# marcottelab/FluorosequencingImageAnalysis

Hardware: AMD Instinct MI355X
Metric: psf_lm_fits_per_sec (higher is better)
Workload: dtype f64

## Files before the change

fluorosequencingimageanalysis_amd/csrc/fsq_fit_rounds.hip:

```cpp
#include <algorithm>
#include <atomic>
#include <cstdlib>

#include <mutex>
#include <new>
#include <type_traits>
#include <vector>

#include "fsq_common.h"
#include "fsq_lm_quad.h"
#include "fsq_evalguard.h"
#include "fsq_kb_tilemap.h"

namespace {

#define WAVE_SYNC() do { __builtin_amdgcn_fence(__ATOMIC_RELEASE, "wavefront"); __builtin_amdgcn_wave_barrier(); \
                         __builtin_amdgcn_fence(__ATOMIC_ACQUIRE, "wavefront"); } while (0)

#ifdef FSQ_DEBUG_HZ
__device__ unsigned long long g_hz[32];
#endif
#ifdef FSQ_PHASE_PROFILE
__device__ unsigned long long g_rphase[32];
#define RPH_DECL unsigned long long rph_t0 = clock64(), rph_acc[16] = {0,0,0,0,0,0,0,0,0,0,0,0,0,0,0,0};
#define RPH_MARK(k) { unsigned long long t_ = clock64(); rph_acc[k] += t_ - rph_t0; rph_t0 = t_; }
#define RPH_FLUSH(off) if (threadIdx.x == 0 && (blockIdx.x & 63) == 0) { for (int k_ = 0; k_ < 16; k_++) atomicAdd(&g_rphase[(off) + k_], rph_acc[k_]); }
#else
#define RPH_DECL
#define RPH_MARK(k)
#define RPH_FLUSH(off)
#endif

enum { CNT_LINE = 32, CNT_A = 0, CNT_B0 = CNT_LINE, CNT_C1 = CNT_B0 + KB_C1 * CNT_LINE, CNT_C3 = CNT_B0 + KB_C3 * CNT_LINE,
       CNT_KINDS = 1 + KB_LISTS, CNT_SET = 8 * CNT_LINE };
__host__ __device__ inline int cnt_of_list(int list) { return CNT_B0 + list * CNT_LINE; }
enum { Q_EPS = Q_WA3 };
enum { A_IDX = 0, A_X = 1, A_DIAG = 8, A_LLIM1 = 15, A_FNORM = 16, A_PAR = 17, A_DELTA = 18, A_XNORM = 19, A_ITER = 20,
       A_HDR = 21 , A_E = 21 , A_LEN = 46,
       B_GNORM = 21, B_IPVT = 22, B_QTF = 23, B_SDIAG = 30, B_R = 37, B_LEN = 65,
       C_PARL = 65, C_PARU = 66, C_FP = 67, C_LMIT = 68, C_LEN = 69 };

struct FitOut {
    double x[FSQ_NP];
    int status, niter, nfev, pad;
};
struct FitStat {
    double vmax, vmean;
};

struct Ctx {
    uint16_t* roi;
    int pix32;
    FitOut* out;
    FitStat* stat;
    long long cap;
    long long pool;
    int* err;
    int* slow_total;
    int* done;
    int tshift;
    int wave_prio;
    int force_redo;
    int force_slow_mod;
};

enum { G_KINIT_POS = 1, G_KINIT_SLOT = 2, G_KA_B = 3, G_KA_OVERLAP = 5, G_KA_SLOW = 6, G_KB_C1 = 7, G_KB_C3 = 8, G_KB_A = 9,
       G_KB_B = 10 };
FSQ_DEV long long fsq_guard(const Ctx& c, long long v, long long limit, int code)
{
    if ((unsigned long long)v < (unsigned long long)limit) return v;
    atomicMax(c.err, code);
    return 0;
}

FSQ_DEV int wave_reserve(int* counter, bool want)
{
    const unsigned long long m = __ballot(want);
    if (m == 0) return 0;
    const int lane = threadIdx.x & 63;
    const int leader = __ffsll((long long)m) - 1;
    int base = 0;
    if (lane == leader) base = atomicAdd(counter, __popcll(m));
    base = __shfl(base, leader);
    return base + __popcll(m & ((1ull << lane) - 1ull));
}

FSQ_DEV int wave_reserve4(int* counters, bool want, int list, int* other)
{
    const int lane = threadIdx.x & 63;
    unsigned long long m[4];
#pragma unroll
    for (int l = 0; l < 4; l++) m[l] = __ballot(want && list == l);
    const unsigned long long mine = list == 0 ? m[0] : list == 1 ? m[1] : list == 2 ? m[2] : m[3];
    const unsigned long long pair = list == 0 ? m[1] : list == 1 ? m[0] : list == 2 ? m[3] : m[2];
    const int leader = want ? __ffsll((long long)mine) - 1 : lane;
    int base = 0;
    if (want && lane == leader) base = atomicAdd(counters + list * CNT_LINE, __popcll(mine));
    const int pair_base = __shfl(base, pair ? __ffsll((long long)pair) - 1 : lane);
    base = __shfl(base, leader);
    *other = pair ? pair_base + __popcll(pair) : 0;
    return want ? base + __popcll(mine & ((1ull << lane) - 1ull)) : 0;
}

FSQ_DEV long long wave_reserve_checked(const Ctx& c, int* counter, bool want, long long limit, int code)
{
    const int at = wave_reserve(counter, want);
    return want ? fsq_guard(c, at, limit, code) : 0;
}

struct BatchArgs {
    const uint16_t* src; const int32_t* cand; int H, W; long long n; int from_image;
    int pix_fmt;
    long long base;
    int ticket;
    int no_queue;
};

FSQ_DEV void wave_mark_done(int* done, bool term, int ticket)
{
    unsigned long long m = __ballot(term);
    const int lane = threadIdx.x & 63;
    while (m) {
        const int leader = __ffsll((long long)m) - 1;
        const int t = __shfl(ticket, leader);
        const unsigned long long mm = __ballot(term && ticket == t);
        if (lane == leader) atomicAdd(done + t, __popcll(mm));
        m &= ~mm;
    }
}

#ifndef FSQ_NT
#define FSQ_NT 0
#endif
typedef unsigned fsq_u4v __attribute__((ext_vector_type(4)));
FSQ_DEV double nt_ld(const double* p) { return FSQ_NT ? __builtin_nontemporal_load(p) : *p; }
FSQ_DEV void nt_st(double* p, double v) { if (FSQ_NT) __builtin_nontemporal_store(v, p); else *p = v; }
FSQ_DEV uint4 nt_ld4(const void* p)
{
    const fsq_u4v v = FSQ_NT ? __builtin_nontemporal_load((const fsq_u4v*)p) : *(const fsq_u4v*)p;
    return make_uint4(v.x, v.y, v.z, v.w);
}
FSQ_DEV void nt_st4(void* p, uint4 w)
{
    fsq_u4v v; v.x = w.x; v.y = w.y; v.z = w.z; v.w = w.w;
    if (FSQ_NT) __builtin_nontemporal_store(v, (fsq_u4v*)p); else *(fsq_u4v*)p = v;
}
struct NtRef {
    double* p;
    FSQ_DEV operator double() const { return nt_ld(p); }
    FSQ_DEV void operator=(double v) const { nt_st(p, v); }
};
struct NtQ {
    double* p;
    FSQ_DEV NtRef operator[](long long i) const { return NtRef{p + i}; }
};
FSQ_DEV NtQ ntq(const double* p) { return NtQ{const_cast<double*>(p)}; }

FSQ_DEV int tag_slot(const Ctx& c, int tag) { return (int)((unsigned)tag & ((1u << c.tshift) - 1u)); }
FSQ_DEV int tag_ticket(const Ctx& c, int tag) { return (int)((unsigned)tag >> c.tshift); }

FSQ_DEV int rpk(int i, int k) { return i * 7 - (i * (i - 1)) / 2 + (k - i); }
FSQ_DEV double pack2(int a, int b) { return __longlong_as_double(((long long)(unsigned)a) | ((long long)b << 32)); }
FSQ_DEV void unpack2(double v, int* a, int* b) { long long u = __double_as_longlong(v); *a = (int)(unsigned)(u & 0xffffffffll); *b = (int)(u >> 32); }

FSQ_DEV void roi_pixels(const BatchArgs& c, long long idx, double* d)
{
    if (c.from_image) {
        const int f = c.cand[3 * idx], h = c.cand[3 * idx + 1], w = c.cand[3 * idx + 2];
        const size_t base = ((size_t)f * c.H + (h - 2)) * c.W + (w - 2);
#pragma unroll
        for (int a = 0; a < 5; a++)
#pragma unroll
            for (int b = 0; b < 5; b++) d[a * 5 + b] = (double)fsq_pixel(c.src, base + (size_t)a * c.W + b, c.pix_fmt);
    } else {
#pragma unroll
        for (int k = 0; k < FSQ_NPIX; k++) d[k] = (double)c.src[idx * FSQ_NPIX + k];
    }
}

FSQ_DEV void roi_compact(const Ctx& c, long long idx, double* d)
{
    if (c.pix32) {
        const uint32_t* s32 = (const uint32_t*)c.roi + (size_t)idx * 32;
#pragma unroll
        for (int k = 0; k < FSQ_NPIX; k++) d[k] = (double)s32[k];
        return;
    }
    const uint16_t* src = c.roi + (size_t)idx * 32;
    const uint4 a = nt_ld4(src), b = nt_ld4(src + 8), e = nt_ld4(src + 16), f = nt_ld4(src + 24);
    const unsigned w[16] = {a.x, a.y, a.z, a.w, b.x, b.y, b.z, b.w, e.x, e.y, e.z, e.w, f.x, f.y, f.z, f.w};
#pragma unroll
    for (int k = 0; k < FSQ_NPIX; k++) d[k] = (double)((w[k >> 1] >> (16 * (k & 1))) & 0xffffu);
}

__global__ void __launch_bounds__(256) kinit(Ctx c, BatchArgs b, double* __restrict__ QA, int* __restrict__ cntA)
{
    const long long i0 = (long long)blockIdx.x * blockDim.x + threadIdx.x;
    const bool ok = i0 < b.n;
    const long long i = ok ? i0 : 0;
    const long long pos = wave_reserve_checked(c, cntA, ok && !b.no_queue, c.cap, G_KINIT_POS);
    if (b.n <= 0) return;
    const long long slot = fsq_guard(c, b.base + i, c.pool, G_KINIT_SLOT);
    double v[FSQ_NPIX];
    roi_pixels(b, i, v);
    if (ok && c.pix32) {
        uint32_t* dst = (uint32_t*)c.roi + (size_t)slot * 32;
#pragma unroll
        for (int k = 0; k < 32; k++) dst[k] = (k < FSQ_NPIX) ? (unsigned)v[k] : 0u;
    } else if (ok) {
        unsigned w[16];
#pragma unroll
        for (int k = 0; k < 16; k++) {
            unsigned lo = (2 * k < FSQ_NPIX) ? (unsigned)v[2 * k] : 0u, hi = (2 * k + 1 < FSQ_NPIX) ? (unsigned)v[2 * k + 1] : 0u;
            w[k] = lo | (hi << 16);
        }
        uint16_t* dst = c.roi + (size_t)slot * 32;
        nt_st4(dst, make_uint4(w[0], w[1], w[2], w[3])); nt_st4(dst + 8, make_uint4(w[4], w[5], w[6], w[7]));
        nt_st4(dst + 16, make_uint4(w[8], w[9], w[10], w[11])); nt_st4(dst + 24, make_uint4(w[12], w[13], w[14], w[15]));
    }
    double mx = v[0], isum = 0.0;
#pragma unroll
    for (int k = 0; k < FSQ_NPIX; k++) { mx = v[k] > mx ? v[k] : mx; isum += v[k]; }
#pragma unroll
    for (int pass = 0; pass < FSQ_NPIX; pass++)
#pragma unroll
        for (int k = (pass & 1); k + 1 < FSQ_NPIX; k += 2) {
            double a = v[k], b_ = v[k + 1];
            v[k] = a < b_ ? a : b_;
            v[k + 1] = a < b_ ? b_ : a;
        }
    if (!ok) return;
    const double vmedian = v[12], vmean = isum / 25.0;
    const double llim1 = (mx - vmean) / 3.0;
    double x0[FSQ_NP] = {vmedian, mx, 2.5, 2.5, 1., 1., 0.};
    c.stat[slot].vmax = mx; c.stat[slot].vmean = vmean;
#pragma unroll
    for (int k = 0; k < FSQ_NP; k++) {
        double t = x0[k];
        if (t > fsq_ulim(k) && fsq_qulim(k)) t = fsq_ulim(k);
        if (t < fsq_llim(k, llim1)) t = fsq_llim(k, llim1);
        x0[k] = t;
    }
    if (b.no_queue) {
#pragma unroll
        for (int k = 0; k < FSQ_NP; k++) c.out[slot].x[k] = x0[k];
        return;
    }
    const NtQ q = ntq(QA + pos);
    const long long cap = c.cap;
#pragma unroll
    for (int k = 0; k < FSQ_NP; k++) {
        q[(A_X + k) * cap] = x0[k];
        q[(A_DIAG + k) * cap] = 0.;
    }
    q[A_IDX * cap] = pack2((int)((unsigned)slot | ((unsigned)b.ticket << c.tshift)), 0);
    q[A_LLIM1 * cap] = llim1; q[A_FNORM * cap] = 0.; q[A_PAR * cap] = 0.; q[A_DELTA * cap] = 0.; q[A_XNORM * cap] = 0.;
    q[A_ITER * cap] = pack2(1, 0);
}

#include "fsq_fit_f32.h"

FSQ_DEV bool fsq_square_is_pow2(double t, double sq, double lo)
{
    const int ex = fsq_expo(sq);
    const double thr = __builtin_ldexp(0.485, ex - 53);
    const bool ok = (__builtin_fabs(lo) <= thr) && ((fsq_bits(sq) & 0xfffffffffffffull) != 0ull) && (sq >= 0x1p-300) && (sq < 0x1p300);
    return ok || (t == 0);
}

template <bool FAST>
FSQ_DEV double gauss_usq(double n, const FsqDivisor& k)
{
    if (FAST) return fsq_sq_of_quotient_ranges_proved(n, k);
    const double q = n / k.d;
    return q * q;
}
template <bool FAST>
FSQ_DEV double gauss_exp(double e) { return FAST ? fsq_exp_bf_unchecked(e) : fsq_exp(e); }
template <bool FAST>
FSQ_DEV double ka_gauss(double nu, double nv, const FsqDivisor& k4, const FsqDivisor& k5)
{
    return gauss_exp<FAST>(-(gauss_usq<FAST>(nu, k4) + gauss_usq<FAST>(nv, k5)) / 2.);
}

#pragma push_macro("QL")
#undef QL
#define QL(off, e) lds[((off) + (e)) * G + grp]
template <int G>
FSQ_DEV double kag_dot7(const double* lds, int grp, int off)
{
    double d = 0.0;
#pragma unroll
    for (int i = 0; i < 7; i++) { double v = QL(off, i); d = fsq_fma(v, v, d); }
    return d;
}
template <int G>
FSQ_DEV double kag_dot25(const double* lds, int grp, int off)
{
    double S[4];
#pragma unroll
    for (int l = 0; l < 4; l++) {
        double a = QL(off, l), b = QL(off, 4 + l), c = QL(off, 8 + l), e = QL(off, 12 + l);
        S[l] = ((a * a + b * b) + c * c) + e * e;
    }
    double d = (S[0] + S[2]) + (S[1] + S[3]);
#pragma unroll
    for (int i = 16; i < 25; i++) { double v = QL(off, i); d = fsq_fma(v, v, d); }
    return d;
}

#define KA_ROWS(i) do { if (L == 8 && ((i) % 5) == 4) __builtin_amdgcn_sched_barrier(0); } while (0)
#define KA_EVAL_LOOP _Pragma("unroll EVAL_UNROLL")
#define KA_PIN(v) do { if (FAST) asm volatile("" : "+v"(v)); } while (0)
#ifdef FSQ_DEBUG_HZ
#define KA_HZ(code, cond) do { if (cond) { hz = true; if (FAST) atomicAdd(&g_hz[code], 1ull); } } while (0)
#else
#define KA_HZ(code, cond) do { if (cond) hz = true; } while (0)
#endif
#ifndef FSQ_KA_QR_STATIC
#define FSQ_KA_QR_STATIC 1
#endif
template <class T> struct ka_step_of { static constexpr int value = -1; };
template <int J> struct ka_step_of<std::integral_constant<int, J>> { static constexpr int value = J; };
template <bool FAST, int L, bool P32 = false, int QRS = 0>
__global__ void __launch_bounds__(64, (L == 8 ? 4 : 2)) kA_jacobian(Ctx c, const double* __restrict__ QA, const int* __restrict__ cntA_p,
                                                                    double* __restrict__ QB, int* __restrict__ cnt_cur,
                                                                    double* __restrict__ SQ, int* __restrict__ slow_cnt,
                                                                    int* __restrict__ next_counters)
{
    constexpr int G = 64 / L;
    constexpr int NC = 8 / L;
    constexpr int MPX = (FSQ_NPIX + L - 1) / L;
    constexpr int MREC = (A_HDR + L - 1) / L;
    constexpr bool EVAL_ALL = FAST && L == 4;
    constexpr int EVAL_UNROLL = EVAL_ALL ? MPX : 1;
    static_assert(QRS == 0 || (FAST && L == 4 && QRS <= 2), "static qrfac steps: the fast four-lane kernel only");
    static_assert(fsq_llim(4, 0.) == FSQ_EG_MIN_SIGMA && fsq_llim(5, 0.) == FSQ_EG_MIN_SIGMA, "fsq_evalguard.h: sigma floor != the fit's lower limit");
    __shared__ double lds[Q_KA_END * G];
    const int lane = threadIdx.x, grp = lane / L, cl = lane % L, gbase = lane - cl;
    const int n7 = FSQ_NP;
    if (c.wave_prio) __builtin_amdgcn_s_setprio(3);
    const int cntA = FAST ? *cntA_p : *slow_cnt;
    if (!FAST && blockIdx.x == 0 && threadIdx.x == 0 && cntA > 0) atomicAdd(c.slow_total, cntA);
    if (FAST && blockIdx.x == 0 && threadIdx.x < CNT_KINDS) next_counters[threadIdx.x * CNT_LINE] = 0;
    double col[NC][FSQ_NPIX];
    RPH_DECL
    const long long cap = c.cap;
    const int stride = gridDim.x * G;
    int base = blockIdx.x * G;
    if (base >= cntA) return;
    do {
        RPH_MARK(0)
        const bool active = (base + grp) < cntA;
        const NtQ qa = ntq(QA + (active ? base + grp : 0));
        double rec[MREC];
#pragma unroll
        for (int m = 0; m < MREC; m++) { const int f = cl + L * m; rec[m] = (active && f < A_HDR) ? (double)qa[f * cap] : 0.0; }
        bool hz = false, qhz = false;
        int emin = 0;
        int tag, niter, nfev, hist;
        unpack2(__shfl(rec[A_IDX / L], gbase + A_IDX % L), &tag, &hist);
        unpack2(__shfl(rec[A_ITER / L], gbase + A_ITER % L), &niter, &nfev);
        const int blist = kb_list_of_history(hist);
        int at_pair;
        const int at_mine = wave_reserve4(cnt_cur + CNT_B0, active && cl == 0, blist, &at_pair);
        if (active && cl == 0) {
            if ((long long)at_mine + (long long)at_pair + 2 > cap && (at_mine > 0 || at_pair > 0)) {
                if ((long long)at_mine + 1 + cnt_cur[cnt_of_list(blist ^ 1)] > cap) atomicMax(c.err, (int)G_KA_OVERLAP);
            }
        }
        const long long at = __shfl((active && cl == 0) ? (int)kb_list_pos(blist, fsq_guard(c, at_mine, cap, G_KA_B), cap) : 0, gbase)
                             + (long long)kb_list_array(blist) * (B_LEN * cap);
        const int idx = tag_slot(c, tag);
        const bool fresh = active && (nfev == 0);
        double llim1 = 0., fnorm = 0., xnorm = 0., delta = 0., par_in = 0.;
        unsigned ipvt = 0x76543210u;
        int status = 0;
        double gnorm = 0.;
        uint4 roi = make_uint4(0u, 0u, 0u, 0u);
        uint4 roi_hi = make_uint4(0u, 0u, 0u, 0u);
        double ev[MPX];
#pragma unroll
        for (int m = 0; m < MPX; m++) ev[m] = 0.0;
        if (active) {
            if (P32) {
                static_assert(!P32 || L == 4, "32-bit pixels: the four-lane Jacobian round only");
                const uint32_t* r32 = (const uint32_t*)c.roi + (size_t)idx * 32 + cl * 8;
                roi = nt_ld4(r32); roi_hi = nt_ld4(r32 + 4);
            } else if (L == 4) roi = nt_ld4(c.roi + (size_t)idx * 32 + cl * 8);
            else {
                const unsigned long long w8 = fsq_bits(nt_ld((const double*)(c.roi + (size_t)idx * 32 + cl * 4)));
                roi.x = (unsigned)w8; roi.y = (unsigned)(w8 >> 32);
            }
            if (!fresh) {
#pragma unroll
                for (int m = 0; m < MPX; m++) { const int k = cl + L * m; if (k < FSQ_NPIX) ev[m] = qa[(A_E + k) * cap]; }
            }
#pragma unroll
            for (int m = 0; m < MREC; m++) {
                const int f = cl + L * m;
                if (f >= 1 && f <= 19) QL(Q_X, f - 1) = rec[m];
            }
        }
        WAVE_SYNC();
        RPH_MARK(1)
        if (active) {
            double xx[FSQ_NP], hh[FSQ_NP];
#pragma unroll
            for (int k = 0; k < FSQ_NP; k++) {
                xx[k] = QL(Q_X, k);
                const double eps = 1.4901161193847656e-08;
                double h_ = eps * __builtin_fabs(xx[k]);
                if (h_ == 0) h_ = eps;
                const double ul = k < 2 ? 0.0 : k < 4 ? 3.0 : k < 6 ? 2.0 : 360.0;
                if (k >= 2 && (xx[k] > ul - h_)) h_ = -h_;
                hh[k] = h_;
            }
            double sn, cs;
            fsq_sincos(FSQ_PI_180 * xx[6], &sn, &cs);
            const double rcx = xx[3] * cs - xx[2] * sn, rcy = xx[3] * sn + xx[2] * cs;
            const FsqDivisor k4 = fsq_divisor(xx[4]), k5 = fsq_divisor(xx[5]);
            if (FAST)
                hz = hz || !fsq_divisor_in_range(xx[4]) || !fsq_divisor_in_range(xx[5]) || !(__builtin_fabs(xx[2]) <= 0x1p100) ||
                     !(__builtin_fabs(xx[3]) <= 0x1p100);
            if (FAST) KA_HZ(15, !fsq_evalguard_ok(cs, sn, rcx, rcy, xx[4], xx[5]));
            {
                const unsigned w[4] = {roi.x, roi.y, roi.z, roi.w};
                const unsigned w32[8] = {roi.x, roi.y, roi.z, roi.w, roi_hi.x, roi_hi.y, roi_hi.z, roi_hi.w};
#pragma unroll
                for (int t = 0; t < 32 / L; t++) {
                    const int k = cl * (32 / L) + t;
                    if (k < FSQ_NPIX) QL(Q_DATA, k) = P32 ? (double)w32[t & 7] : (double)((w[t >> 1] >> (16 * (t & 1))) & 0xffffu);
                }
                if (!fresh) {
#pragma unroll
                    for (int m = 0; m < MPX; m++) { const int k = cl + L * m; if (k < FSQ_NPIX) QL(Q_FVEC, k) = ev[m]; }
                }
            }
            WAVE_SYNC();
            if (__ballot(fresh)) {
                if (fresh) {
                    KA_EVAL_LOOP
                    for (int m = 0; m < MPX; m++) {
                        const int i = EVAL_ALL ? min(cl + L * m, FSQ_NPIX - 1) : cl + L * m;
                        if (EVAL_ALL || i < FSQ_NPIX) {
                            const int xi = i / 5;
                            const double x = (double)xi, y = (double)(i - 5 * xi);
                            const double xp = x * cs - y * sn, yp = x * sn + y * cs;
                            const double E = ka_gauss<FAST>(rcx - xp, rcy - yp, k4, k5);
                            QL(Q_FVEC, i) = E;
                        }
                    }
                }
                WAVE_SYNC();
            }
            if (fresh) nfev = 1;
            {
                const double x2p = xx[2] + hh[2], x3p = xx[3] + hh[3];
                const double rcx2 = xx[3] * cs - x2p * sn, rcy2 = xx[3] * sn + x2p * cs;
                const double rcx3 = x3p * cs - xx[2] * sn, rcy3 = x3p * sn + xx[2] * cs;
                if (FAST) KA_HZ(0, !(__builtin_fabs(x2p) <= 0x1p100) || !(__builtin_fabs(x3p) <= 0x1p100));
                if (FAST) KA_HZ(15, !fsq_eg_centre_ok(rcx2, rcy2) || !fsq_eg_centre_ok(rcx3, rcy3));
                KA_EVAL_LOOP
                for (int m = 0; m < MPX; m++) {
                    const int i = EVAL_ALL ? min(cl + L * m, FSQ_NPIX - 1) : cl + L * m;
                    if (EVAL_ALL || i < FSQ_NPIX) {
                        const int xi = i / 5;
                        const double x = (double)xi, y = (double)(i - 5 * xi);
                        const double xp = x * cs - y * sn, yp = x * sn + y * cs;
                        const double d = QL(Q_DATA, i);
                        const double E2 = ka_gauss<FAST>(rcx2 - xp, rcy2 - yp, k4, k5);
                        const double E3 = ka_gauss<FAST>(rcx3 - xp, rcy3 - yp, k4, k5);
                        QL(Q_STAGE, i) = d - (xx[0] + xx[1] * E2);
                        QL(Q_STAGE + 25, i) = d - (xx[0] + xx[1] * E3);
                    }
                }
                const double p0 = (cl == 0) ? xx[0] + hh[0] : xx[0], p1 = (cl == 1) ? xx[1] + hh[1] : xx[1];
#pragma unroll
                for (int i = 0; i < FSQ_NPIX; i++) { col[0][i] = QL(Q_DATA, i) - (p0 + p1 * QL(Q_FVEC, i)); KA_ROWS(i); }
                WAVE_SYNC();
                if (cl == 2 || cl == 3) {
#pragma unroll
                    for (int i = 0; i < FSQ_NPIX; i++) { col[0][i] = QL(Q_STAGE + 25 * (cl - 2), i); KA_ROWS(i); }
                }
                double fvm[MPX];
#pragma unroll
                for (int m = 0; m < MPX; m++) {
                    const int i = cl + L * m;
                    fvm[m] = (i < FSQ_NPIX) ? QL(Q_DATA, i) - (xx[0] + xx[1] * QL(Q_FVEC, i)) : 0.0;
                }
                WAVE_SYNC();
#pragma unroll
                for (int m = 0; m < MPX; m++) {
                    const int i = cl + L * m;
                    if (i < FSQ_NPIX) QL(Q_FVEC, i) = fvm[m];
                }
            }
            {
                const double x4p = xx[4] + hh[4], x5p = xx[5] + hh[5];
                const FsqDivisor k4p = fsq_divisor(x4p), k5p = fsq_divisor(x5p);
                double snt, cst;
                fsq_sincos(FSQ_PI_180 * (xx[6] + hh[6]), &snt, &cst);
                const double rcxt = xx[3] * cst - xx[2] * snt, rcyt = xx[3] * snt + xx[2] * cst;
                if (FAST) KA_HZ(1, !fsq_divisor_in_range(x4p) || !fsq_divisor_in_range(x5p));
                if (FAST) KA_HZ(15, !fsq_eg_sigma_ok(x4p) || !fsq_eg_sigma_ok(x5p) || !fsq_eg_rotation_ok(cst, snt) || !fsq_eg_centre_ok(rcxt, rcyt));
                KA_EVAL_LOOP
                for (int m = 0; m < MPX; m++) {
                    const int i = EVAL_ALL ? min(cl + L * m, FSQ_NPIX - 1) : cl + L * m;
                    if (EVAL_ALL || i < FSQ_NPIX) {
                        const int xi = i / 5;
                        const double x = (double)xi, y = (double)(i - 5 * xi);
                        const double xp = x * cs - y * sn, yp = x * sn + y * cs;
                        const double nu = rcx - xp, nv = rcy - yp;
                        const double ub2 = gauss_usq<FAST>(nu, k4), vb2 = gauss_usq<FAST>(nv, k5);
                        const double u42 = gauss_usq<FAST>(nu, k4p), v52 = gauss_usq<FAST>(nv, k5p);
                        const double E4 = gauss_exp<FAST>(-(u42 + vb2) / 2.);
                        const double E5 = gauss_exp<FAST>(-(ub2 + v52) / 2.);
                        const double xpt = x * cst - y * snt, ypt = x * snt + y * cst;
                        const double Et = ka_gauss<FAST>(rcxt - xpt, rcyt - ypt, k4, k5);
                        const double d = QL(Q_DATA, i);
                        QL(Q_STAGE, i) = d - (xx[0] + xx[1] * E4);
                        QL(Q_STAGE + 25, i) = d - (xx[0] + xx[1] * E5);
// ... 328 lines not shown
                if (REGPOS) {
                    double dj = QL(Q_TMP, 5);
                    if (broken) dj = pos_get(prd[0], prd[1], j);
                    QL(Q_R, j * 7 + lj) = dj;
                } else {
                    if (!broken) QL(Q_RDIAG, j) = QL(Q_TMP, 5);
                    QL(Q_R, j * 7 + lj) = QL(Q_RDIAG, j);
                }
                if (!ST) {
#pragma unroll
                    for (int pass = 0; pass < (CMP ? 1 : NC); pass++) {
#pragma unroll
                        for (int i = 0; i + 1 < FSQ_NPIX; i++) col[pass][i] = col[pass][i + 1];
                        col[pass][FSQ_NPIX - 1] = 0.0;
                    }
                }
                WAVE_SYNC();
                RPH_MARK(11)
            };
#define KA_STEP(J, CMPV) qr_step(std::integral_constant<int, J>{}, std::integral_constant<bool, CMPV>{})
            if constexpr (QRS == 2) { KA_STEP(0, false); KA_STEP(1, false); KA_STEP(2, false); }
            else
                for (int j = 0; j < (COMPACT ? 3 : n7); j++) qr_step(j, std::false_type{});
            if constexpr (QRS != 0) { KA_STEP(3, true); KA_STEP(4, true); KA_STEP(5, true); KA_STEP(6, true); }
            else if (COMPACT)
                for (int j = 3; j < n7; j++) qr_step(j, std::true_type{});
#undef KA_STEP
            RPH_MARK(4)
#define QRG(i, k) QL(Q_R, (i) * 7 + nib_get(ipvt, (k)))
            llim1 = QL(Q_TMP, 0); fnorm = QL(Q_TMP, 1); par_in = QL(Q_TMP, 2); delta = QL(Q_TMP, 3); xnorm = QL(Q_TMP, 4);
            if (niter == 1) {
#pragma unroll
                for (int k = 0; k < FSQ_NP; k++) {
                    double a = QL(Q_ACN, k);
                    double dg = (a == 0) ? 1. : a;
                    QL(Q_DIAG, k) = dg;
                    QL(Q_WA3, k) = dg * QL(Q_X, k);
                }
                xnorm = fsq_sqrt(kag_dot7<G>(lds, grp, Q_WA3));
                delta = 100. * xnorm;
                if (delta == 0.) delta = 100.;
            }
            gnorm = 0.;
            if (fnorm != 0) {
                for (int j = 0; j < n7; j++) {
                    double an = QL(Q_ACN, nib_get(ipvt, j));
                    if (an != 0) {
                        double sg = 0.0;
                        for (int i = 0; i <= j; i++) sg += QRG(i, j) * QL(Q_QTF, i);
                        sg = sg / fnorm;
                        gnorm = np_max2(gnorm, __builtin_fabs(sg / an));
                    }
                }
            }
            if (gnorm <= 1e-10) status = 4;
            else {
#pragma unroll
                for (int k = 0; k < FSQ_NP; k++) { double dg = QL(Q_DIAG, k), an = QL(Q_ACN, k); QL(Q_DIAG, k) = (dg > an) ? dg : an; }
            }
            RPH_MARK(5)
            if (FAST) {
                KA_HZ(13, (emin < -FSQ_DIV_EN));
                if (c.force_slow_mod > 0 && (idx % c.force_slow_mod) == 0) hz = true;
                const unsigned long long m = __ballot(hz);
                qhz = ((m >> gbase) & ((1ull << L) - 1ull)) != 0;
            }
            if (status != 0 && cl == 0 && !qhz) {
                FitOut o;
#pragma unroll
                for (int k = 0; k < FSQ_NP; k++) o.x[k] = QL(Q_X, k);
                o.status = status; o.niter = niter; o.nfev = nfev; o.pad = 0;
                c.out[idx] = o;
            }
        }
        wave_mark_done(c.done, active && status != 0 && cl == 0 && !qhz, tag_ticket(c, tag));
        {
            bool go = active && (status == 0);
            if (FAST) {
                int sat = (int)wave_reserve_checked(c, slow_cnt, qhz && cl == 0, cap, G_KA_SLOW);
                sat = __shfl(sat, gbase);
                if (qhz) for (int f = cl; f < A_LEN; f += L) nt_st(SQ + (size_t)sat + f * cap, qa[f * cap]);
                go = go && !qhz;
            }
            const NtQ qb = ntq(QB + at);
            if (go) {
                for (int e = cl; e < 28; e += L) {
                    int i = 0, rem = e;
                    while (rem >= 7 - i) { rem -= 7 - i; i++; }
                    qb[(B_R + e) * cap] = QRG(i, i + rem);
                }
                for (int k = cl; k < FSQ_NP; k += L) {
                    qb[(A_X + k) * cap] = QL(Q_X, k);
                    qb[(A_DIAG + k) * cap] = QL(Q_DIAG, k);
                    qb[(B_QTF + k) * cap] = QL(Q_QTF, k);
                    qb[(B_SDIAG + k) * cap] = 0.;
                }
                if (cl == 0) {
                    qb[A_IDX * cap] = pack2(tag, hist);
                    qb[A_LLIM1 * cap] = llim1; qb[A_FNORM * cap] = fnorm; qb[A_PAR * cap] = par_in; qb[A_DELTA * cap] = delta;
                    qb[A_XNORM * cap] = xnorm; qb[A_ITER * cap] = pack2(niter, nfev);
                    qb[B_GNORM * cap] = gnorm; qb[B_IPVT * cap] = pack2((int)ipvt, 0);
                }
            } else if (active && cl == 0) qb[A_IDX * cap] = pack2(-1, 0);
        }
        RPH_MARK(6)
        base += stride;
    } while (!FAST && base < cntA);
    RPH_FLUSH(16)
}
#undef QRG
#undef REFL
#undef KA_ROWS
#undef KA_PIN
#undef KA_EVAL_LOOP
#undef KA_HZ
#pragma pop_macro("QL")

#ifndef FSQ_KA_LANES_DEFAULT
#define FSQ_KA_LANES_DEFAULT 4
#endif
#ifndef FSQ_LMPAR_LIMITS
#define FSQ_LMPAR_LIMITS {0, 3, 3, 10, 3, 10}
#endif
#ifndef FSQ_KB_WAVES
#define FSQ_KB_WAVES 2
#endif
FSQ_DEV int kb_res_slot(int i) { return i < 14 ? i : i + 7; }

template <bool FAST>
FSQ_DEV bool kb_trial_gauss(const double* p, double* myscr)
{
    bool bad = false;
    double s, c;
    fsq_sincos(FSQ_PI_180 * p[6], &s, &c);
    const double rcen_x = p[3] * c - p[2] * s;
    const double rcen_y = p[3] * s + p[2] * c;
    const FsqDivisor k4 = fsq_divisor(p[4]), k5 = fsq_divisor(p[5]);
    if (FAST)
        bad = !fsq_divisor_in_range(p[4]) || !fsq_divisor_in_range(p[5]) || !(__builtin_fabs(p[2]) <= 0x1p100) ||
              !(__builtin_fabs(p[3]) <= 0x1p100) || !fsq_evalguard_ok(c, s, rcen_x, rcen_y, p[4], p[5]);
#pragma unroll 1
    for (int xi = 0; xi < 5; xi++) {
        const double x = (double)xi;
#pragma unroll
        for (int yi = 0; yi < 5; yi++) {
            const double y = (double)yi;
            const double xp = x * c - y * s;
            const double yp = x * s + y * c;
            const double nu = rcen_x - xp, nv = rcen_y - yp;
            myscr[kb_res_slot(xi * 5 + yi) * 64] = ka_gauss<FAST>(nu, nv, k4, k5);
        }
    }
    return bad;
}

FSQ_DEV double kb_late_load(const NtRef r) { asm volatile("" ::: "memory"); return (double)r; }

struct KbLimits { int lim[KB_LISTS]; };
template <bool ALIASED, bool P32 = false>
__global__ void __launch_bounds__(64, FSQ_KB_WAVES) kB_step(Ctx c, const double* __restrict__ QB, const double* __restrict__ QC,
                                                  const int* __restrict__ cnt_cur,
                                                  double* __restrict__ QA_next, double* __restrict__ QB_next, double* __restrict__ QC_next,
                                                  int* __restrict__ cnt_next, KbLimits lims)
{
    __shared__ double scr[32 * 64];
    if (c.wave_prio) __builtin_amdgcn_s_setprio(3);
// ... 207 lines not shown
            wa3[j] = 0;
            double wj = myscr[(14 + nib_get(ipvt, j)) * 64];
#pragma unroll
            for (int i = 0; i < FSQ_NP; i++)
                if (i <= j) wa3[i] = wa3[i] + q.r[i][j] * wj;
        }
        double t1s = 0.0;
#pragma unroll
        for (int k = 0; k < FSQ_NP; k++) { double t = alpha * wa3[k]; t1s = fsq_fma(t, t, t1s); }
        double temp1 = fsq_sqrt(t1s) / fnorm;
        double temp2 = (fsq_sqrt(alpha * par) * pnorm) / fnorm;
        double prered = temp1 * temp1 + (temp2 * temp2) / 0.5;
        double dirder = -(temp1 * temp1 + temp2 * temp2);
        double ratio = 0.;
        if (prered != 0) ratio = actred / prered;
        if (ratio <= 0.25) {
            double temp;
            if (actred >= 0) temp = .5;
            else temp = .5 * dirder / (dirder + .5 * actred);
            if (((0.1 * fnorm1) >= fnorm) || (temp < 0.1)) temp = 0.1;
            delta = temp * np_min2(delta, pnorm / 0.1);
            par = par / temp;
        } else if ((par == 0) || (ratio >= 0.75)) {
            delta = pnorm / .5;
            par = .5 * par;
        }
        const bool accepted = (ratio >= 0.0001);
        if (accepted) {
            double xs = 0.0;
#pragma unroll
            for (int k = 0; k < FSQ_NP; k++) {
                xq[k] = wa2[k];
                double t = q.dg[k] * wa2[k];
                xs = fsq_fma(t, t, xs);
            }
            xnorm = fsq_sqrt(xs);
            fnorm = fnorm1;
            niter = niter + 1;
        }
        int status = 0;
        bool c1 = (__builtin_fabs(actred) <= 1e-10) && (prered <= 1e-10) && (0.5 * ratio <= 1);
        if (c1) status = 1;
        if (delta <= 1e-10 * xnorm) status = 2;
        if (c1 && (status == 2)) status = 3;
        if (status == 0) {
            if (niter >= 200) status = 5;
            if ((__builtin_fabs(actred) <= FSQ_MACHEP) && (prered <= FSQ_MACHEP) && (0.5 * ratio <= 1)) status = 6;
            if (delta <= FSQ_MACHEP * xnorm) status = 7;
            if (KB_GNORM() <= FSQ_MACHEP) status = 8;
        }
        if (status == 0 && !accepted) {
            bool fin = __builtin_isfinite(ratio);
#pragma unroll
            for (int k = 0; k < FSQ_NP; k++)
                fin = fin && __builtin_isfinite(wa1[k]) && __builtin_isfinite(wa2[k]) && __builtin_isfinite(xq[k]);
            if (!fin) status = -16;
        }
        RPH_MARK(5)
        if (live && status != 0) {
            FitOut o;
#pragma unroll
            for (int k = 0; k < FSQ_NP; k++) o.x[k] = xq[k];
            o.status = status; o.niter = niter; o.nfev = nfev; o.pad = 0;
            c.out[tag_slot(c, tag)] = o;
        }
        wave_mark_done(c.done, live && status != 0, tag_ticket(c, tag));
        {
            const bool toA = live && status == 0 && accepted, toB = live && status == 0 && !accepted;
            const int blist = kb_list_of_history(lm_hist);
            const int atA = (int)wave_reserve_checked(c, cnt_next + CNT_A, toA, cap, G_KB_A);
            int atB_pair;
            const int atB = wave_reserve4(cnt_next + CNT_B0, toB, blist, &atB_pair);
            if (toA || toB) {
                const NtQ qn = ntq(toA ? (QA_next + atA)
                                       : (QB_next + (long long)kb_list_array(blist) * (B_LEN * cap) + kb_list_pos(blist, fsq_guard(c, atB, cap, G_KB_B), cap)));
                qn[A_IDX * cap] = pack2(tag, lm_hist);
#pragma unroll
                for (int k = 0; k < FSQ_NP; k++) { qn[(A_X + k) * cap] = xq[k]; qn[(A_DIAG + k) * cap] = q.dg[k]; }
                qn[A_LLIM1 * cap] = llim1; qn[A_FNORM * cap] = fnorm; qn[A_PAR * cap] = par; qn[A_DELTA * cap] = delta;
                qn[A_XNORM * cap] = xnorm; qn[A_ITER * cap] = pack2(niter, nfev);
                if (toA) {
#pragma unroll
                    for (int i = 0; i < FSQ_NPIX; i++) qn[(A_E + i) * cap] = myscr[kb_res_slot(i) * 64];
                }
                if (toB) {
                    qn[B_GNORM * cap] = KB_GNORM(); qn[B_IPVT * cap] = pack2((int)ipvt, 0);
#pragma unroll
                    for (int k = 0; k < FSQ_NP; k++) { qn[(B_QTF + k) * cap] = q.qtf[k]; qn[(B_SDIAG + k) * cap] = q.sdiag[k]; }
#undef KB_GNORM
#pragma unroll
                    for (int i = 0; i < FSQ_NP; i++)
#pragma unroll
                        for (int k = i; k < FSQ_NP; k++) qn[(B_R + rpk(i, k)) * cap] = q.r[i][k];
                }
            }
        }
        RPH_MARK(6)
    }
    RPH_FLUSH(0)
}

__global__ void __launch_bounds__(64) kfinish(Ctx c, BatchArgs b, FsqRow* __restrict__ rows)
{
    long long i = (long long)blockIdx.x * blockDim.x + threadIdx.x;
    if (i >= b.n) return;
    const long long slot = b.base + i;
    const FitOut S = c.out[slot];
    double data[FSQ_NPIX], p[FSQ_NP];
    roi_compact(c, slot, data);
#pragma unroll
    for (int k = 0; k < FSQ_NP; k++) p[k] = S.x[k];
    const double vmax = c.stat[slot].vmax, vmean = c.stat[slot].vmean;
    int h = 2, w = 2, field = 0;
    if (b.from_image) { field = b.cand[3 * i]; h = b.cand[3 * i + 1]; w = b.cand[3 * i + 2]; }
    double fit[FSQ_NPIX];
    fsq_model(p, fit);
    double num = 0.0, den = 0.0, rm = 0.0;
    for (int k = 0; k < FSQ_NPIX; k++) { double d = data[k] - fit[k]; num += d * d; }
    for (int k = 0; k < FSQ_NPIX; k++) { double d = data[k] - vmean; den += d * d; }
    for (int k = 0; k < FSQ_NPIX; k++) rm += fsq_pow2(data[k] - fit[k]);
    FsqRow r;
    r.h0 = p[2] + h - 2.5;
    r.w0 = p[3] + w - 2.5;
    r.H = p[0]; r.A = p[1]; r.sigma_h = p[4]; r.sigma_w = p[5]; r.theta = p[6];
    r.rmse = fsq_sqrt(rm / 25.0);
    r.r2 = 1.0 - num / den;
    {
        double op[16];
        int t = 0;
        for (int ww = 0; ww < 5; ww++) op[t++] = data[ww];
        for (int ww = 0; ww < 5; ww++) op[t++] = data[20 + ww];
        for (int hh = 1; hh < 4; hh++) { op[t++] = data[hh * 5]; op[t++] = data[hh * 5 + 4]; }
        double isum = 0.0;
        for (int k = 0; k < 16; k++) isum += op[k];
        double mean = isum / 16.0, rr[8];
        for (int k = 0; k < 8; k++) { double d0 = op[k] - mean, d1 = op[8 + k] - mean; rr[k] = d0 * d0 + d1 * d1; }
        double res = ((rr[0] + rr[1]) + (rr[2] + rr[3])) + ((rr[4] + rr[5]) + (rr[6] + rr[7]));
        res = 0.0 + res;
        r.s_n = (vmax - mean) / fsq_sqrt(res / 16.0);
    }
    r.p2 = p[2]; r.p3 = p[3];
    r.h = h; r.w = w; r.field = field;
    const int status = S.status;
    r.status = status; r.niter = S.niter; r.nfev = S.nfev + (status > 0 ? 1 : 0);
    r.key_h = -1; r.key_w = -1;
    rows[i] = r;
}

}

namespace {
__global__ void kdivcheck(const double* __restrict__ num, const double* __restrict__ den, long long n, unsigned long long* bad)
{
    long long i = (long long)blockIdx.x * blockDim.x + threadIdx.x;
    if (i >= n) return;
    const double a = num[i], d = den[i];
    const FsqDivisor k = fsq_divisor(d);
    const double q0 = a / d, q1 = fsq_div_by(a, k);
    if (fsq_bits(q0) != fsq_bits(q1)) atomicAdd(bad, 1ull);
}
std::atomic<long long> g_last_slow{0};

__global__ void ksqcheck(const double* __restrict__ t, long long n, unsigned long long* bad)
{
    long long i = (long long)blockIdx.x * blockDim.x + threadIdx.x;
    if (i >= n) return;
// ... 573 lines not shown
```

Baseline: 24.22 million.

## Carry ROI pixels in A-queue records and prefetch next record speculatively

Adds eight packed ROI words to each A-queue record, written by the init kernel and by the round that re-queues to A. The A-round then reads pixels from the record instead of gathering through the tag-indexed ROI pool. The A-round kernel also loads its first record (header, residuals, ROI) before the early-exit check, and splits the B-slot atomic reservation into issue and finish halves so its latency can overlap other work. The cost is a longer A record, extra stores when re-queuing to A, and a speculative load that can be wasted.

```diff
diff --git a/fluorosequencingimageanalysis_amd/csrc/fsq_fit_rounds.hip b/fluorosequencingimageanalysis_amd/csrc/fsq_fit_rounds.hip
--- a/fluorosequencingimageanalysis_amd/csrc/fsq_fit_rounds.hip
+++ b/fluorosequencingimageanalysis_amd/csrc/fsq_fit_rounds.hip
@@ -35,8 +35,15 @@
        CNT_KINDS = 1 + KB_LISTS, CNT_SET = 8 * CNT_LINE };
 __host__ __device__ inline int cnt_of_list(int list) { return CNT_B0 + list * CNT_LINE; }
 enum { Q_EPS = Q_WA3 };
+#ifndef FSQ_KA_SPEC
+#define FSQ_KA_SPEC 1
+#endif
+#ifndef FSQ_KA_ROIREC
+#define FSQ_KA_ROIREC 1
+#endif
 enum { A_IDX = 0, A_X = 1, A_DIAG = 8, A_LLIM1 = 15, A_FNORM = 16, A_PAR = 17, A_DELTA = 18, A_XNORM = 19, A_ITER = 20,
-       A_HDR = 21 , A_E = 21 , A_LEN = 46,
+       A_HDR = 21 , A_E = 21 ,
+       A_ROI = 46 , A_LEN = FSQ_KA_ROIREC ? 54 : 46,
        B_GNORM = 21, B_IPVT = 22, B_QTF = 23, B_SDIAG = 30, B_R = 37, B_LEN = 65,
        C_PARL = 65, C_PARU = 66, C_FP = 67, C_LMIT = 68, C_LEN = 69 };
 
@@ -85,7 +92,19 @@
     return base + __popcll(m & ((1ull << lane) - 1ull));
 }
 
-FSQ_DEV int wave_reserve4(int* counters, bool want, int list, int* other)
+FSQ_DEV int wave_reserve4_issue(int* counters, bool want, int list)
+{
+    const int lane = threadIdx.x & 63;
+    unsigned long long m[4];
+#pragma unroll
+    for (int l = 0; l < 4; l++) m[l] = __ballot(want && list == l);
+    const unsigned long long mine = list == 0 ? m[0] : list == 1 ? m[1] : list == 2 ? m[2] : m[3];
+    const int leader = want ? __ffsll((long long)mine) - 1 : lane;
+    int base = 0;
+    if (want && lane == leader) base = atomicAdd(counters + list * CNT_LINE, __popcll(mine));
+    return base;
+}
+FSQ_DEV int wave_reserve4_finish(int base, bool want, int list, int* other)
 {
     const int lane = threadIdx.x & 63;
     unsigned long long m[4];
@@ -94,12 +113,14 @@
     const unsigned long long mine = list == 0 ? m[0] : list == 1 ? m[1] : list == 2 ? m[2] : m[3];
     const unsigned long long pair = list == 0 ? m[1] : list == 1 ? m[0] : list == 2 ? m[3] : m[2];
     const int leader = want ? __ffsll((long long)mine) - 1 : lane;
-    int base = 0;
-    if (want && lane == leader) base = atomicAdd(counters + list * CNT_LINE, __popcll(mine));
     const int pair_base = __shfl(base, pair ? __ffsll((long long)pair) - 1 : lane);
     base = __shfl(base, leader);
     *other = pair ? pair_base + __popcll(pair) : 0;
     return want ? base + __popcll(mine & ((1ull << lane) - 1ull)) : 0;
+}
+FSQ_DEV int wave_reserve4(int* counters, bool want, int list, int* other)
+{
+    return wave_reserve4_finish(wave_reserve4_issue(counters, want, list), want, list, other);
 }
 
 FSQ_DEV long long wave_reserve_checked(const Ctx& c, int* counter, bool want, long long limit, int code)
@@ -144,6 +165,15 @@
 {
     fsq_u4v v; v.x = w.x; v.y = w.y; v.z = w.z; v.w = w.w;
     if (FSQ_NT) __builtin_nontemporal_store(v, (fsq_u4v*)p); else *(fsq_u4v*)p = v;
+}
+FSQ_DEV unsigned long long nt_ld_bits(const double* p)
+{
+    return FSQ_NT ? __builtin_nontemporal_load((const unsigned long long*)p) : *(const unsigned long long*)p;
+}
+FSQ_DEV void nt_st_bits(double* p, unsigned lo, unsigned hi)
+{
+    const unsigned long long v = (unsigned long long)lo | ((unsigned long long)hi << 32);
+    if (FSQ_NT) __builtin_nontemporal_store(v, (unsigned long long*)p); else *(unsigned long long*)p = v;
 }
 struct NtRef {
     double* p;
@@ -213,6 +243,10 @@
         for (int k = 0; k < 16; k++) {
             unsigned lo = (2 * k < FSQ_NPIX) ? (unsigned)v[2 * k] : 0u, hi = (2 * k + 1 < FSQ_NPIX) ? (unsigned)v[2 * k + 1] : 0u;
             w[k] = lo | (hi << 16);
+        }
+        if (FSQ_KA_ROIREC && !b.no_queue) {
+#pragma unroll
+            for (int k = 0; k < 8; k++) nt_st_bits(QA + pos + (long long)(A_ROI + k) * c.cap, w[2 * k], w[2 * k + 1]);
         }
         uint16_t* dst = c.roi + (size_t)slot * 32;
         nt_st4(dst, make_uint4(w[0], w[1], w[2], w[3])); nt_st4(dst + 8, make_uint4(w[4], w[5], w[6], w[7]));
@@ -348,6 +382,19 @@
     const long long cap = c.cap;
     const int stride = gridDim.x * G;
     int base = blockIdx.x * G;
+    constexpr bool SPEC = FAST && (FSQ_KA_SPEC != 0);
+    constexpr bool ROIREC = (FSQ_KA_ROIREC != 0) && L == 4 && !P32;
+    double srec[MREC], sev[MPX];
+    unsigned long long sroi[2] = {0ull, 0ull};
+    if (SPEC) {
+        const long long sp = (long long)(base + grp) < cap - 1 ? (long long)(base + grp) : cap - 1;
+        const NtQ qs = ntq(QA + sp);
+#pragma unroll
+        for (int m = 0; m < MREC; m++) { const int f = cl + L * m; srec[m] = (f < A_HDR) ? (double)qs[f * cap] : 0.0; }
+        if (ROIREC) { sroi[0] = nt_ld_bits(QA + sp + (A_ROI + 2 * cl) * cap); sroi[1] = nt_ld_bits(QA + sp + (A_ROI + 2 * cl + 1) * cap); }
+#pragma unroll
+        for (int m = 0; m < MPX; m++) { const int k = cl + L * m; sev[m] = (k < FSQ_NPIX) ? (double)qs[(A_E + k) * cap] : 0.0; }
+    }
     if (base >= cntA) return;
     do {
         RPH_MARK(0)
@@ -355,22 +402,32 @@
         const NtQ qa = ntq(QA + (active ? base + grp : 0));
         double rec[MREC];
 #pragma unroll
-        for (int m = 0; m < MREC; m++) { const int f = cl + L * m; rec[m] = (active && f < A_HDR) ? (double)qa[f * cap] : 0.0; }
+        for (int m = 0; m < MREC; m++) {
+            const int f = cl + L * m;
+            if (SPEC) rec[m] = active ? srec[m] : 0.0;
+            else rec[m] = (active && f < A_HDR) ? (double)qa[f * cap] : 0.0;
+        }
         bool hz = false, qhz = false;
         int emin = 0;
         int tag, niter, nfev, hist;
         unpack2(__shfl(rec[A_IDX / L], gbase + A_IDX % L), &tag, &hist);
         unpack2(__shfl(rec[A_ITER / L], gbase + A_ITER % L), &niter, &nfev);
         const int blist = kb_list_of_history(hist);
-        int at_pair;
-        const int at_mine = wave_reserve4(cnt_cur + CNT_B0, active && cl == 0, blist, &at_pair);
-        if (active && cl == 0) {
-            if ((long long)at_mine + (long long)at_pair + 2 > cap && (at_mine > 0 || at_pair > 0)) {
-                if ((long long)at_mine + 1 + cnt_cur[cnt_of_list(blist ^ 1)] > cap) atomicMax(c.err, (int)G_KA_OVERLAP);
-            }
-        }
-        const long long at = __shfl((active && cl == 0) ? (int)kb_list_pos(blist, fsq_guard(c, at_mine, cap, G_KA_B), cap) : 0, gbase)
-                             + (long long)kb_list_array(blist) * (B_LEN * cap);
+        constexpr bool LATE_SLOT = SPEC && (FSQ_KA_SPEC >= 2);
+        const int at_raw = wave_reserve4_issue(cnt_cur + CNT_B0, active && cl == 0, blist);
+        auto b_slot = [&]() __attribute__((always_inline)) {
+            int at_pair;
+            const int at_mine = wave_reserve4_finish(at_raw, active && cl == 0, blist, &at_pair);
+            if (active && cl == 0) {
+                if ((long long)at_mine + (long long)at_pair + 2 > cap && (at_mine > 0 || at_pair > 0)) {
+                    if ((long long)at_mine + 1 + cnt_cur[cnt_of_list(blist ^ 1)] > cap) atomicMax(c.err, (int)G_KA_OVERLAP);
+                }
+            }
+            return __shfl((active && cl == 0) ? (int)kb_list_pos(blist, fsq_guard(c, at_mine, cap, G_KA_B), cap) : 0, gbase)
+                   + (long long)kb_list_array(blist) * (B_LEN * cap);
+        };
+        long long at = 0;
+        if (!LATE_SLOT) at = b_slot();
         const int idx = tag_slot(c, tag);
         const bool fresh = active && (nfev == 0);
         double llim1 = 0., fnorm = 0., xnorm = 0., delta = 0., par_in = 0.;
@@ -387,6 +444,10 @@
                 static_assert(!P32 || L == 4, "32-bit pixels: the four-lane Jacobian round only");
                 const uint32_t* r32 = (const uint32_t*)c.roi + (size_t)idx * 32 + cl * 8;
                 roi = nt_ld4(r32); roi_hi = nt_ld4(r32 + 4);
+            } else if (ROIREC) {
+                const unsigned long long w0 = SPEC ? sroi[0] : nt_ld_bits(qa.p + (A_ROI + 2 * cl) * cap);
+                const unsigned long long w1 = SPEC ? sroi[1] : nt_ld_bits(qa.p + (A_ROI + 2 * cl + 1) * cap);
+                roi = make_uint4((unsigned)w0, (unsigned)(w0 >> 32), (unsigned)w1, (unsigned)(w1 >> 32));
             } else if (L == 4) roi = nt_ld4(c.roi + (size_t)idx * 32 + cl * 8);
             else {
                 const unsigned long long w8 = fsq_bits(nt_ld((const double*)(c.roi + (size_t)idx * 32 + cl * 4)));
@@ -394,7 +455,7 @@
             }
             if (!fresh) {
 #pragma unroll
-                for (int m = 0; m < MPX; m++) { const int k = cl + L * m; if (k < FSQ_NPIX) ev[m] = qa[(A_E + k) * cap]; }
+                for (int m = 0; m < MPX; m++) { const int k = cl + L * m; if (k < FSQ_NPIX) ev[m] = SPEC ? sev[m] : (double)qa[(A_E + k) * cap]; }
             }
 #pragma unroll
             for (int m = 0; m < MREC; m++) {
@@ -438,6 +499,7 @@
                 }
             }
             WAVE_SYNC();
+            RPH_MARK(12)
             if (__ballot(fresh)) {
                 if (fresh) {
                     KA_EVAL_LOOP
@@ -932,6 +994,7 @@
                 if (qhz) for (int f = cl; f < A_LEN; f += L) nt_st(SQ + (size_t)sat + f * cap, qa[f * cap]);
                 go = go && !qhz;
             }
+            if (LATE_SLOT) at = b_slot();
             const NtQ qb = ntq(QB + at);
             if (go) {
                 for (int e = cl; e < 28; e += L) {
@@ -1305,6 +1368,15 @@
                 if (toA) {
 #pragma unroll
                     for (int i = 0; i < FSQ_NPIX; i++) qn[(A_E + i) * cap] = myscr[kb_res_slot(i) * 64];
+                    if (FSQ_KA_ROIREC && !P32) {
+                        const uint16_t* src = c.roi + (size_t)tag_slot(c, tag) * 32;
+#pragma unroll
+                        for (int g = 0; g < 4; g++) {
+                            const uint4 v = nt_ld4(src + 8 * g);
+                            nt_st_bits(qn.p + (A_ROI + 2 * g) * cap, v.x, v.y);
+                            nt_st_bits(qn.p + (A_ROI + 2 * g + 1) * cap, v.z, v.w);
+                        }
+                    }
                 }
                 if (toB) {
                     qn[B_GNORM * cap] = KB_GNORM(); qn[B_IPVT * cap] = pack2((int)ipvt, 0);
```

Result: slower. 23.78 million (-1.8%).
